# doing-science-to-stuff/ndt

Measured on AMD Instinct MI355X. Metric: Mray/s (primary+shadow+reflect) at 1920x1080, higher is better.
Workload: dtype f64

## Files before the change

### ndt_amd/csrc/ndt_device.hpp

```cpp
#pragma once
#include <hip/hip_runtime.h>
#include <stdint.h>

#define NDT_EPS   (1e-4)
#define NDT_EPS2  ((NDT_EPS) * (NDT_EPS))
#define NDT_INV_EPS2 (1.0 / (NDT_EPS2))
#define NDT_DBL_MAX 1.7976931348623157e308
#define NDT_PI 3.14159265358979323846

#define NDT_DEV __device__ __forceinline__

#define NDT_F_TYPE_MASK   0xff
#define NDT_F_GATE        0x100
#define NDT_F_INF_ENDS    0x200
#define NDT_F_USE_NORMALS 0x400
#define NDT_F_TRANSPARENT 0x800
#define NDT_F_BOX         0x1000
#define NDT_F_FACEBOX     0x2000
#define NDT_F_OBOX        0x4000
#define NDT_F_FACETREE    0x8000
#define NDT_F_FACEGROUPS  0x10000

enum { T_SPHERE = 0, T_HPLANE, T_HDISK, T_CYLINDER, T_HCYLINDER, T_ORTHOTOPE, T_HCUBE, T_HFACET, T_FACET };
enum { NDT_LIGHT_AMBIENT_ = 0, NDT_LIGHT_POINT_ = 1, NDT_LIGHT_DIRECTIONAL_ = 2, NDT_LIGHT_SPOT_ = 3 };
// ... 1116 lines not shown
            } else {
#pragma unroll
                for (int c = 0; c < N; ++c) {
                    w2[c].x = blob[src + 2 * c];
                    w2[c].y = blob[src + 2 * c + 1];
                }
            }
            l_ref[lane] = ref;
            if (has_box) l_ord[lane] = blob[sd.off_oord + id];
            const long long h0 = __double_as_longlong(hdr.x), h1 = __double_as_longlong(hdr.y);
            l_inf[lane] = __longlong_as_double(((h0 >> 32) & 0xffffffffll) | (((h1 & 0xffffll) | ((h1 >> 32) << 16)) << 32));
#pragma unroll
            for (int c = 0; c < N; ++c) *reinterpret_cast<ndt_v2d *>(l_win + lane * 2 * N + 2 * c) = w2[c];
        }
        cls_lds_sync();
        NDT_STAMP(4);
        unsigned long long seen = 0ull;
        if (open && mask.hist_n > 0) {
            for (int k0 = 0; k0 < cnt; k0 += 8) {
                int ids[8];
#pragma unroll
                for (int j = 0; j < 8; ++j) ids[j] = (int)(__double_as_longlong(l_ref[(k0 + j < cnt) ? k0 + j : cnt - 1]) & 0xffffffffll);
                seen |= (unsigned long long)mask.seen_of_8(ids) << k0;
            }
        }
        unsigned long long want = 0ull, any = 0ull;
        if (__ballot(open != 0) != 0ull) {
            unsigned long long todo = (cnt < 64) ? ((1ull << cnt) - 1ull) : ~0ull;
            if (beam) {
                bool keep = true;
                if (lane < cnt && (((int)(__double_as_longlong(l_ref[lane]) >> 32)) & NDT_F_OBOX)) {
                    const unsigned long long ord = (unsigned long long)__double_as_longlong(l_ord[lane]);
                    double t0 = 0.0, t1 = NDT_DBL_MAX;
#pragma unroll
                    for (int k = 0; k < N; ++k) {
                        const int axis = (int)((ord >> (4 * k)) & 15ull);
                        const ndt_v2d box = *reinterpret_cast<const ndt_v2d *>(l_win + lane * 2 * N + 2 * k);
                        const double x0 = l_beam[4 * axis], i0 = l_beam[4 * axis + 1], i1 = l_beam[4 * axis + 2];
                        if (l_beam[4 * axis + 3] != 0.0) {
                            const double a = x0 - box.x, h = box.y;
                            const double p = -h - a, q = h - a;
                            const double c1 = p * i0, c2 = p * i1, c3 = q * i0, c4 = q * i1;
                            const double lo12 = c1 < c2 ? c1 : c2, lo34 = c3 < c4 ? c3 : c4;
                            const double hi12 = c1 < c2 ? c2 : c1, hi34 = c3 < c4 ? c4 : c3;
                            const double lo = lo12 < lo34 ? lo12 : lo34, hi = hi12 > hi34 ? hi12 : hi34;
                            if (lo > t0) t0 = lo;
                            if (hi < t1) t1 = hi;
                        }
                    }
                    keep = t0 <= t1;
                }
                todo &= __ballot(keep);
            }
            while (todo != 0ull) {
                const int k = __ffsll((long long)todo) - 1;
                todo &= todo - 1ull;
                const int flags = __builtin_amdgcn_readfirstlane((int)(__double_as_longlong(l_ref[k]) >> 32));
                bool pass = open != 0;
                if (flags & NDT_F_OBOX) {
                    if (open) pass = item_box_meets<N>(l_win, sd_win, k, box_slot);
                } else if (flags & NDT_F_GATE) {
                    SceneDesc sd_sph = sd;
                    sd_sph.off_bs = k * (2 * N) - k * (N + 2);
                    if (open) pass = bsphere_gate<N>(l_win, sd_sph, k, o, v, min_dist);
                }
                if (pass) want |= 1ull << k;
                if (__ballot(pass && !((seen >> k) & 1ull)) != 0ull) any |= 1ull << k;
            }
            want &= ~seen;
        }
        NDT_STAMP(7);
        int cur = 0;
        auto record_of = [&](int k, int &flags, int &words, int &m, int &at, int &sph) {
            const long long ibits = __double_as_longlong(l_inf[k]);
            const int wm = __builtin_amdgcn_readfirstlane((int)(ibits >> 32));
            at = sd.off_params + __builtin_amdgcn_readfirstlane((int)(ibits & 0xffffffffll));
            words = (wm & 0xffff) + N + 2;
            m = wm >> 16;
            const long long rbits = __double_as_longlong(l_ref[k]);
            flags = __builtin_amdgcn_readfirstlane((int)(rbits >> 32));
            sph = sd.off_bs + __builtin_amdgcn_readfirstlane((int)(rbits & 0xffffffffll)) * (N + 2);
        };
        auto word_of = [&](int j, int words, int at, int sph) {
            return (j < words) ? blob[(j < N + 2) ? sph + j : at + j - (N + 2)] : 0.0;
        };
        auto put = [&](double *buf, int flags, int words, int m, double t0, double t1) {
            if (lane < words) buf[2 + lane] = t0;
            if (lane + 64 < words) buf[2 + 64 + lane] = t1;
            if (lane == 0) {
                buf[0] = __longlong_as_double((long long)(unsigned int)flags);
                buf[1] = __longlong_as_double((long long)m << 32);
            }
        };
        if (any != 0ull) {
            int flags, words, m, at, sph;
            record_of(__ffsll((long long)any) - 1, flags, words, m, at, sph);
            const double t0 = word_of(lane, words, at, sph), t1 = word_of(lane + 64, words, at, sph);
            put(l_par, flags, words, m, t0, t1);
            cls_lds_sync();
        }
        while (any != 0ull) {
            const int k = __ffsll((long long)any) - 1;
            any &= any - 1ull;
            int n_flags = 0, n_words = 0, n_m = 0, n_at = 0, n_sph = 0;
            double t0 = 0.0, t1 = 0.0;
            if (any != 0ull) {
                record_of(__ffsll((long long)any) - 1, n_flags, n_words, n_m, n_at, n_sph);
                t0 = word_of(lane, n_words, n_at, n_sph);
                t1 = word_of(lane + 64, n_words, n_at, n_sph);
            }
            const long long rbits = __double_as_longlong(l_ref[k]);
            const int id = __builtin_amdgcn_readfirstlane((int)(rbits & 0xffffffffll));
            const int flags = __builtin_amdgcn_readfirstlane((int)(rbits >> 32));
            const double *rec = l_par + cur * par_stride;
            bool pass = open != 0 && ((want >> k) & 1ull);
            if ((flags & NDT_F_GATE) && pass) pass = bsphere_gate<N>(rec, sd_par, 0, o, v, min_dist);
            if (pass) {
                double res[N], nrm[N];
                if (isect<N, false>(rec, sd_par, 0, o, v, res, nrm)) {
                    const double dist = v_dist<N>(o, res);
                    if (dist > NDT_EPS && (dist + NDT_EPS < min_dist || min_dist < 0)) {
                        min_dist = dist;
                        best = id;
                    }
                    if (dist_limit == 0.0 || dist < dist_limit) {
                        open = 0;
                        last = id;
                    }
                }
            }
            cur ^= 1;
            if (any != 0ull) put(l_par + cur * par_stride, n_flags, n_words, n_m, t0, t1);
            cls_lds_sync();
            if (__ballot(open != 0) == 0ull) any = 0ull;
        }
        cls_lds_sync();
        NDT_STAMP(2);
        if (open) last = (int)(__double_as_longlong(l_ref[cnt - 1]) & 0xffffffffll);
        cls_lds_sync();
    }
}

#define NDT_KD_STACK 40
#define NDT_STACK_FLAG 0x40000000



struct KdStackLds {
    double *tu;
    int *node;
    int stride;
};

template <int N, int MW, bool LSTACK = false, bool UNI = false>
NDT_DEV void trace_kd(const double *blob, const SceneDesc &sd, VisitMask<MW> &mask, const double (&o)[N],
                      const double (&v)[N], double dist_limit, int &out_obj, int &out_prim
#ifdef NDT_PHASE_TIMING
                      , unsigned long long (&ph)[8], unsigned int (&cnt)[8], unsigned int (&occ)[8]
#endif
                      , KdStackLds ls = KdStackLds{}, ClsLds cl = ClsLds{}, const bool has_ray = true, double *box_slot = nullptr)
{
#ifdef NDT_PHASE_TIMING
    unsigned long long ph_last = __builtin_readcyclecounter();
#endif
#ifdef NDT_T1_KEEP_INV
    constexpr bool KEEP_INV = true;
#else
    constexpr bool KEEP_INV = (MW != 0);
#endif
    auto inv_of = [](double v_i) {
        double r;
        if (v_i < NDT_EPS2 && v_i >= 0.0)
            r = NDT_INV_EPS2;
        else if (v_i > -NDT_EPS2 && v_i <= 0.0)
            r = -NDT_INV_EPS2;
        else
            r = 1.0 / v_i;
        return r;
    };
    double v_inv[N];
    if (KEEP_INV) {
#pragma unroll
        for (int i = 0; i < N; ++i) v_inv[i] = inv_of(v[i]);
    }
    auto inv_at = [&](int dim) {
        if constexpr (KEEP_INV) return v_pick<N>(v_inv, dim);
        else return inv_of(v_pick<N>(v, dim));
    };
    NDT_STAMP(5);

    double t_inf = NDT_DBL_MAX;
    int inf_obj = -1, inf_prim = -1;
    double lt = NDT_DBL_MAX;
    int l_obj = -1, l_prim = -1;

    int st_node[LSTACK ? 1 : NDT_KD_STACK];
    double st_a[LSTACK ? 1 : NDT_KD_STACK], st_tu[LSTACK ? 1 : NDT_KD_STACK];
    int sp = 0;
    int node = 0;
    double ntl = 0, ntu = 0;
    int st = 4;
    bool boxed = false;

    constexpr bool BITS = (MW == 1);
    unsigned long long cand = 0ull;
    int sec = 0, pos = 0, end = 0;
    double min_dist = -1;
    int best_obj = -1, best_prim = -1;
    int sub_i = 0, sub_end = 0, sub_owner = -1, sub_prim = -1;
    long long sub_live = -1;
    double sub_min = -1;

    if (!has_ray) {
        st = 3;
    } else if (sd.n_inf > 0) {
        st = 5;
        if (BITS) {
            cand = sd.inf_bits;
        } else {
            sec = sd.off_inf;
            pos = 0;
            end = sd.n_inf;
        }
    }

    while (true) {
        if (st == 4) {
            double tl = -NDT_DBL_MAX, tu = NDT_DBL_MAX;
            bool box = true;
#pragma unroll
            for (int i = 0; i < N; ++i) {
                if (box) {
                    double v_i = v[i], o_i = o[i];
                    if (!(fabs(v_i) < NDT_EPS2)) {
                        double tl_i = (blob[sd.off_bb + i] - o_i) / v_i;
                        double tu_i = (blob[sd.off_bb + N + i] - o_i) / v_i;
                        if (tl_i > tu_i) {
                            double tmp = tl_i;
                            tl_i = tu_i;
                            tu_i = tmp;
                        }
                        if (tl_i > tl) tl = tl_i;
                        if (tu_i < tu) tu = tu_i;
                        if (tu < -NDT_EPS) box = false;
                    }
                }
            }
            if (box) {
                tl -= NDT_EPS;
                tu += NDT_EPS;
                box = (tu >= -NDT_EPS) && (tl <= tu);
            }
            if (!box || sd.n_kd_nodes <= 0) {
                st = 3;
            } else {
                mask.clear(sd.mask_words);
                if (BITS && sd.gate_bits != 0ull) {
                    unsigned long long todo = sd.gate_bits, dead = 0ull;
                    while (todo != 0ull) {
                        const int id = __ffsll((long long)todo) - 1;
                        todo &= todo - 1ull;
                        const int b = sd.off_bs + id * (N + 2);
                        double c[N], oc[N];
                        blob_vec<N>(blob, b, c);
                        v_sub<N>(o, c, oc);
                        const double oc_len2 = v_dot<N>(oc, oc);
                        const double voc = v_dot<N>(v, oc);
                        const double voc2 = voc * voc;
                        const double desc = voc2 - oc_len2 + blob[b + N + 1];
                        if (desc < 0.0 || (voc > 0.0 && voc2 > desc)) dead |= 1ull << id;
                    }
                    mask.w[0] |= dead;
                }
                node = 0;
                ntl = tl;
                ntu = tu;
                st = 1;
            }
        }
        {
            while (st < 2) {
                NDT_OCC(0);
                if (st == 0) {
                    if (sp == 0) {
                        st = 3;
                    } else {
                        sp -= LSTACK ? ls.stride : 1;
                        double a;
                        if (LSTACK) {
                            const int parent = ls.node[sp];
                            ntu = ls.tu[sp];
                            const ndt_v2d prec = blob_pair(blob, sd.off_kd + 2 * parent);
                            const long long pw0 = __double_as_longlong(prec.x);
                            const int pdim = (int)(pw0 & 0xffffffffll);
                            const double pv_inv = inv_at(pdim);
                            a = (prec.y - v_pick<N>(o, pdim)) * pv_inv;
                            node = (pv_inv < NDT_EPS2) ? parent + 1 : (int)(pw0 >> 32);
                        } else {
                            node = st_node[sp];
                            a = st_a[sp];
                            ntu = st_tu[sp];
                        }
                        ntl = a - NDT_EPS;
                        st = ((lt > a) & !(ntu < 0.0)) ? 1 : 0;
                    }
                } else if (ntu < 0.0) {
                    st = 0;
                }
                if (st == 1) {
                    NDT_COUNT(0);
                    ndt_v2d rec = blob_pair(blob, sd.off_kd + 2 * node);
                    unsigned long long below = ~0ull;
                    if (BITS) {
                        double ns = blob[sd.off_nset + node];
#ifndef NDT_NO_T_HOIST
                        asm volatile("" : "+v"(rec.x), "+v"(rec.y), "+v"(ns));
#endif
                        below = (unsigned long long)__double_as_longlong(ns) & ~mask.w[0];
                    }
                    const long long w0 = __double_as_longlong(rec.x);
                    const int dim = (int)(w0 & 0xffffffffll);
                    if (BITS && below == 0ull) {
                        st = 0;
                    } else if (dim < 0) {
                        if (BITS) {
                            st = 2;
                            cand = below;
                        } else {
                            const long long w1 = __double_as_longlong(rec.y);
                            const int num = (int)(w1 >> 32);
                            st = num > 0 ? 2 : 0;
                            sec = sd.off_leaf;
                            pos = (int)(w1 & 0xffffffffll);
                            end = pos + num;
                        }
                    } else {
                        const double boundary = rec.y;
                        const double v_inv_i = inv_at(dim);
                        const double o_i = v_pick<N>(o, dim);
                        const bool swap = v_inv_i < NDT_EPS2;
                        const int left = node + 1, right = (int)(w0 >> 32);
                        const int near = swap ? right : left, far = swap ? left : right;
                        const double tp = (boundary - o_i) * v_inv_i;
                        const bool alive = lt > ntl;
                        const bool near_only = (ntu < tp - NDT_EPS) & alive;
                        const bool far_only = !near_only & (ntl > tp + NDT_EPS) & alive;
                        const bool both = !near_only & !far_only;
                        if (both & (lt > tp)) {
                            if (LSTACK) { ls.node[sp] = node; ls.tu[sp] = ntu; }
                            else { st_node[sp] = far; st_a[sp] = tp; st_tu[sp] = ntu; }
                            sp += LSTACK ? ls.stride : 1;
                        }
                        const bool go_near = near_only | (both & alive);
                        ntu = (both & alive) ? tp + NDT_EPS : ntu;
                        node = go_near ? near : far;
                        st = (go_near | far_only) ? 1 : 0;
                    }
                }
            }
        }
        NDT_STAMP(0);
        const bool have_list = st == 2 || st == 5, list_is_inf = st == 5;
        if (UNI ? (__ballot(have_list) == 0ull) : !have_list) break;

        min_dist = -1;
        best_obj = -1;
        best_prim = -1;
        bool list_open = have_list;
        bool scanned_together = false;
        if (UNI && MW == 0 && cl.base) {
            const bool elig = have_list && !list_is_inf && mask.hist_n >= 0;
            unsigned long long todo = __ballot(elig);
            const int n_listed = __popcll(__ballot(have_list));
            while (todo != 0ull) {
                const int leader = __ffsll((long long)todo) - 1;
                const int w0 = __builtin_amdgcn_readlane(sec + pos, leader), e0 = __builtin_amdgcn_readlane(sec + end, leader);
                bool mine = elig && sec + pos == w0;
                const unsigned long long group = __ballot(mine);
                todo &= ~group;
                if (__popcll(group) < cl.min_group && !(__popcll(group) == n_listed && n_listed >= 16)) mine = false;
                if (__ballot(mine) == 0ull) continue;
                double md;
                int best, last;
                NDT_STAMP(3);
#ifdef NDT_PHASE_TIMING
                cls_scan<N, MW>(blob, sd, mask, cl.base, mine, o, v, dist_limit, w0, e0, box_slot, boxed, md, best, last, ph, ph_last);
#else
                cls_scan<N, MW>(blob, sd, mask, cl.base, mine, o, v, dist_limit, w0, e0, box_slot, boxed, md, best, last);
#endif
                if (mine) {
                    min_dist = md;
                    best_obj = best;
                    best_prim = best;
                    mask.end_leaf(blob_int(blob, sd.off_kd + 2 * node, 1), last);
                    list_open = false;
                    scanned_together = true;
                }
            }
        }
        int gs = list_open ? 0 : 4;
        while (gs != 4) {
            int prim = -1;
            while (gs < 2) {
                NDT_OCC(1);
                if (gs == 1 && sub_live == 0) {
                    const int oflags = blob_int(blob, sd.off_hdr + 2 * sub_owner, 0);
                    const int first = blob_int(blob, sd.off_hdr + 2 * sub_owner + 1, 0);
                    const bool fresh_hcube = sub_i == first;
                    long long live = -1;
                    int chunk = (sub_i - first) / NDT_HULL_CHUNK;
                    if (oflags & NDT_F_BOX)
                        live = hull_faces<N>(blob, sd.off_params + blob_int(blob, sd.off_hdr + 2 * sub_owner, 1),
                                             (oflags & NDT_F_FACEBOX) != 0, sub_end - first, o, v, chunk, (oflags & NDT_F_FACETREE) != 0,
                                             (oflags & NDT_F_FACEGROUPS) != 0);
                    if (live == 0) {
                        if (fresh_hcube) gs = 0;
                        else sub_i = sub_end;
                        sub_live = -1;
                    } else {
                        const int skip = __ffsll(live) - 1;
                        sub_i = first + ((live == -1) ? 0 : chunk * NDT_HULL_CHUNK) + skip;
                        sub_live = live >> skip;
                    }
                }
                if (gs == 1 && sub_i == sub_end) {
// ... 195 lines not shown
```

### ndt_amd/csrc/ndt_kernels.hip

```cpp
#if NDT_DIMS <= 5 && !defined(NDT_OUTLINE_SMALL)
#define NDT_INLINE_LIBM 1
#endif
#if NDT_DIMS <= 7 && !defined(NDT_OUTLINE_SMALL)
#define NDT_SHADE_INLINE_ISECT 1
#endif
#include "ndt_kernels.hpp"
#include <hip/hip_ext.h>
#include <stdlib.h>
#include <map>
#include <mutex>
#include <tuple>

#ifndef NDT_DIMS
#error "compile with -DNDT_DIMS=<3..10>"
#endif
#define NDT_CAT2(a, b) a##b
#define NDT_CAT(a, b) NDT_CAT2(a, b)

namespace NDT_CAT(ndt_d, NDT_DIMS) {

static constexpr int N = NDT_DIMS;


NDT_DEV int wave_excl_scan(int x, int &total)
// ... 90 lines not shown
        } else if (half_j > 1080 + 45) {
            jp = jp - (1080 + 45);
            eye = 2;
        } else {
            prim_sti<COH>(ws.depth_left + g, 0);
            prim_sti<COH>(ws.hit_obj + g, -1);
            return false;
        }
    }
    const double x = ip / (double)rg.img_w - 0.5;
    const double y = -(jp / y_div - 0.5);
    double pixel[N], temp[N], cam[N];
    blob_vec<N>(blob, sd.off_cam, pos);
    const double focal = blob[sd.off_cam + 4 * N];
    const int ext = sd.off_cam + 4 * N + 8;
    const int cam_type = PLANAR ? 0 : (int)blob[ext];
    if (!PLANAR && cam_type != 0) {
        const double azi = x * blob[ext + 1];
        double view_x, view_y, view_z;
        if (cam_type == 1) {
            const double alt = y * blob[ext + 2];
            view_x = focal * sin(azi) * cos(alt);
            view_y = focal * sin(alt);
            view_z = focal * cos(azi) * cos(alt);
        } else {
            const double y_size = 2.0 * tan(blob[ext + 2] / 2.0) * focal;
            view_x = focal * sin(azi);
            view_y = y * y_size;
            view_z = focal * cos(azi);
        }
        double ax[N];
        v_copy<N>(pixel, pos);
        blob_vec<N>(blob, ext + 3 + 2 * N, ax);
        v_scale<N>(ax, view_x, temp);
        v_add<N>(pixel, temp, pixel);
        blob_vec<N>(blob, ext + 3 + 3 * N, ax);
        v_scale<N>(ax, view_y, temp);
        v_add<N>(pixel, temp, pixel);
        blob_vec<N>(blob, ext + 3 + 4 * N, ax);
        v_scale<N>(ax, view_z, temp);
        v_add<N>(pixel, temp, pixel);
    } else {
        double orig[N], dx[N], dy[N];
        blob_vec<N>(blob, sd.off_cam + N, orig);
        blob_vec<N>(blob, sd.off_cam + 2 * N, dx);
        blob_vec<N>(blob, sd.off_cam + 3 * N, dy);
        v_scale<N>(dx, rg.aspect_w / (double)rg.aspect_h, dx);
        v_copy<N>(pixel, orig);
        v_scale<N>(dx, x, temp);
        v_add<N>(pixel, temp, pixel);
        v_scale<N>(dy, y, temp);
        v_add<N>(pixel, temp, pixel);
        const double screen_dist = v_dist<N>(orig, pos);
        if (screen_dist > NDT_EPS) {
            v_sub<N>(pixel, pos, temp);
            v_scale<N>(temp, focal / screen_dist, temp);
            v_add<N>(pos, temp, pixel);
        }
    }
    v_copy<N>(cam, pos);
    if (eye == 0) blob_vec<N>(blob, ext + 3, cam);
    else if (eye == 2) blob_vec<N>(blob, ext + 3 + N, cam);
    if (!PLANAR && cam_type != 0 && eye != 1) {
        const double azi = x * blob[ext + 1];
        double lx[N], lz[N], bx[N], bz[N], local[N], px[N], pz[N];
        blob_vec<N>(blob, ext + 3 + 2 * N, lx);
        blob_vec<N>(blob, ext + 3 + 4 * N, lz);
        v_proj<N>(lx, lz, temp);
        v_sub<N>(lx, temp, bx);
        v_copy<N>(bz, lz);
        v_unitize<N>(bx);
        v_unitize<N>(bz);
        v_sub<N>(cam, pos, local);
        v_proj<N>(local, bx, px);
        v_proj<N>(local, bz, pz);
        const double vx = v_dot<N>(px, bx), vz = v_dot<N>(pz, bz);
        double rx[N], rz[N];
        v_scale<N>(bx, vx * cos(azi) - vz * sin(azi), rx);
        v_scale<N>(bz, vz * cos(azi) + vx * sin(azi), rz);
        v_sub<N>(cam, px, cam);
        v_sub<N>(cam, pz, cam);
        v_add<N>(cam, rx, cam);
        v_add<N>(cam, rz, cam);
    }
    if (rg.samples && rg.lens) {
        double ax[N];
        blob_vec<N>(blob, ext + 3 + 2 * N, ax);
        v_scale<N>(ax, rg.samples[4 * g + 2], temp);
        v_add<N>(cam, temp, cam);
        blob_vec<N>(blob, ext + 3 + 3 * N, ax);
        v_scale<N>(ax, rg.samples[4 * g + 3], temp);
        v_add<N>(cam, temp, cam);
    }
    v_sub<N>(pixel, cam, look);
    v_unitize<N>(look);
    v_copy<N>(pos, cam);
    {
        const long long at = (g >> 6) * (long long)(N * 64) + (g & 63);
#pragma unroll
        for (int c = 0; c < N; ++c) {
            prim_st<COH>(ws.ray_o + at + c * 64, pos[c]);
            prim_st<COH>(ws.ray_v + at + c * 64, look[c]);
        }
    }
    prim_st<COH>(ws.frac + g, 1.0);
    prim_sti<COH>(ws.depth_left + g, rg.max_depth);
    if (rg.samples && rg.sample_keys) prim_stu<COH>(ws.rng_key + g, rg.sample_keys[g]);
    return true;
}

__global__ void __launch_bounds__(256) k_primary(const double *blob, SceneDesc sd, Workspace ws, RenderGeom rg)
{
    const long long g = (long long)blockIdx.x * blockDim.x + threadIdx.x;
    if (g >= rg.n_primary) return;
    double pos[N], look[N];
    (void)primary_node<false>(blob, sd, ws, rg, g, pos, look);
}



NDT_DEV LevelRange *job_levels_mut(const TraceJob &job) { return const_cast<LevelRange *>(job.levels); }

template <int MW> NDT_DEV void init_visit_mask(VisitMask<MW> &mask, const double *gblob, const SceneDesc &sd, const Workspace &ws)
{
    mask.ext = nullptr;
    mask.ext_stride = 0;
    mask.h0 = mask.h1 = mask.h2 = mask.h3 = 0u;
    mask.hist_n = -1;
    mask.slab_words = sd.mask_words;
    mask.ls.sets = nullptr;
    mask.ls.blob = gblob;
    mask.ls.words = sd.mask_words;
    mask.ls.off_lrange = sd.off_lrange;
    mask.ls.off_leaf = sd.off_leaf;
    mask.ls.cap = sd.hist_cap;
    if (MW == 0) {
        const long long lane_slot = (long long)blockIdx.x * blockDim.x + threadIdx.x;
        mask.ext = ws.mask_slab + lane_slot;
        mask.ext_stride = (int)ws.mask_slab_lanes;
        if (sd.off_lset > 0) mask.ls.sets = reinterpret_cast<const unsigned long long *>(gblob + sd.off_lset);
    }
}

NDT_DEV int seg_light_origin(const double *gblob, const SceneDesc &sd, int s)
{
    unsigned long long rest = ~sd.ambient_bits;
    for (int k = 0; k < s; ++k) rest &= rest - 1ull;
    const int li = __ffsll((long long)rest) - 1;
    const int w = sd.off_lights + li * (6 + 4 * N);
    const int type = blob_int(gblob, w, 0);
    return (type == NDT_LIGHT_POINT_ || type == NDT_LIGHT_SPOT_) ? w + 5 : -1;
}

#ifndef NDT_TICKET_AHEAD
#define NDT_TICKET_AHEAD 256
#endif
template <int MW, bool LDS, bool LSTACK = false, bool PRIM = false>
__global__ void __launch_bounds__(MW == 0 ? NDT_TRACE_T1_MAX_BLOCK : NDT_TRACE_MAX_BLOCK) k_trace(const double *__restrict__ gblob, SceneDesc sd, Workspace ws, TraceJob job)
{
    extern __shared__ __attribute__((aligned(16))) double lds_blob[];
    const double *blob = gblob;
    if (LDS) {
        const int pairs = sd.trace_words >> 1;
        const ndt_v2d *src2 = reinterpret_cast<const ndt_v2d *>(gblob);
        ndt_v2d *dst2 = reinterpret_cast<ndt_v2d *>(lds_blob);
        int i = threadIdx.x;
        for (; i + 3 * (int)blockDim.x < pairs; i += 4 * blockDim.x) {
            const ndt_v2d a = src2[i], b = src2[i + blockDim.x], c = src2[i + 2 * blockDim.x], d = src2[i + 3 * blockDim.x];
            dst2[i] = a; dst2[i + blockDim.x] = b; dst2[i + 2 * blockDim.x] = c; dst2[i + 3 * blockDim.x] = d;
        }
        for (; i < pairs; i += blockDim.x) dst2[i] = src2[i];
        if ((sd.trace_words & 1) && threadIdx.x == 0) lds_blob[sd.trace_words - 1] = gblob[sd.trace_words - 1];
        __syncthreads();
        blob = lds_blob;
    }
    KdStackLds kstack{};
    if (LSTACK) {
        double *base = lds_blob + ((sd.trace_words + 1) & ~1);
        const int depth = sd.kd_depth + 1;
        kstack.stride = blockDim.x;
        kstack.tu = base + threadIdx.x;
        kstack.node = (int *)(base + (size_t)depth * blockDim.x) + threadIdx.x;
    }
    VisitMask<MW> mask;
    init_visit_mask<MW>(mask, gblob, sd, ws);
    ClsLds cls{};
    double *box_slot = nullptr;
    if (MW == 0 && !LDS) {
        const int wave = threadIdx.x >> 6, waves = blockDim.x >> 6;
        const int box_words = sd.off_obox > 0 ? N * 128 : 0;
        if (sd.off_obox > 0) box_slot = lds_blob + (size_t)wave * box_words + 2 * (threadIdx.x & 63);
        if (sd.cls_par_words > 0) {
            cls.base = lds_blob + (size_t)waves * box_words + (size_t)wave * cls_window_words<N>(sd.cls_par_words);
            cls.min_group = sd.cls_min_group;
        }
    }
    const int lane = __lane_id();
    const unsigned int probe_start = job.exit_log ? (unsigned int)wall_clock64() : 0u;
    unsigned int probe_batch = probe_start;
#ifdef NDT_PHASE_TIMING
    unsigned long long ph[8] = { 0, 0, 0, 0, 0, 0, 0, 0 };
    unsigned long long acc[24];
    for (int i = 0; i < 24; ++i) acc[i] = 0ull;
    unsigned long long out_last = __builtin_readcyclecounter();
    unsigned long long batch_mark = 0;
#endif
    const int bs = job.batch;
    const int sh = (bs == 64) ? 6 : (bs == 32) ? 5 : (bs == 16) ? 4 : 3;
    int seg_batches = 0, seg_batches_incl = 0, seg_cnt = 0;
    if (job.n_seg > 0) {
        seg_cnt = (lane < job.n_seg) ? job.seg_count[lane] : 0;
        const int excl = wave_excl_scan((seg_cnt + bs - 1) >> sh, seg_batches);
        seg_batches_incl = excl + ((seg_cnt + bs - 1) >> sh);
    }
    long long dense_count = job.count, dense_begin = job.begin, seg_stride = job.seg_stride;
    if (job.levels) {
        const LevelRange cur = job.levels[job.seg_level];
        seg_stride = cur.seg_stride;
        LevelRange next;
        if (job.publish_level >= 0) {
            next.begin = cur.begin + cur.count;
            next.count = (long long)ws.counters[0] - next.begin;
            next.n_shadow = 0;
            if (next.count < 0 || (ws.counters[2] & 1) != 0) next.count = 0;
            next.seg_stride = (next.count + 63) & ~63LL;
            const bool sh_overflow = (long long)job.n_seg * next.seg_stride > ws.sh_cap;
            if (blockIdx.x == 0 && threadIdx.x < 64) {
                long long emitted = seg_cnt;
                for (int d = 32; d > 0; d >>= 1) emitted += __shfl_xor(emitted, d, 64);
                NDT_SEG_COUNTERS(ws, job.publish_level + 1)[lane] = 0;
                if (lane == 0) {
                    job_levels_mut(job)[job.publish_level].n_shadow = emitted;
                    LevelRange out = next;
                    if (sh_overflow) {
                        atomicOr(&ws.counters[2], 2);
                        const long long need = (long long)job.n_seg * next.seg_stride;
                        ws.counters[3] = need > 0x7fffffffLL ? 0x7fffffff : (int)need;
                        out.count = 0;
                        out.seg_stride = 0;
                    }
                    job_levels_mut(job)[job.publish_level + 1] = out;
                    ws.mail[job.publish_level + 1] = out;
                    __threadfence_system();
                    __hip_atomic_store(&ws.mail_tag[job.publish_level + 1], job.publish_tag, __ATOMIC_RELEASE, __HIP_MEMORY_SCOPE_SYSTEM);
                }
            }
            if (sh_overflow) next.count = 0;
        } else {
            next = job.levels[job.dense_level >= 0 ? job.dense_level : 0];
        }
        if (job.dense_level >= 0) {
            dense_begin = next.begin;
            dense_count = next.count;
        } else {
            dense_count = 0;
        }
    }
    const long long dense_batches = (dense_count + bs - 1) >> sh;
    const long long n_batches = dense_batches + seg_batches;
    const int reserve = ((threadIdx.x >> 6) >= 4) ? job.tail_solo : 0;
    int cur = blockIdx.x % NDT_QUEUE_SHARDS;
    long long last_k = -1;
    bool any_left = true;
    int k_ahead = -1;
    while (true) {
        long long b = -1;
        if (k_ahead >= 0) {
            const int k = __shfl(k_ahead, 0, 64);
            const long long n_here = (n_batches - cur + NDT_QUEUE_SHARDS - 1) / NDT_QUEUE_SHARDS;
            k_ahead = -1;
            if (k < n_here) {
                b = (long long)k * NDT_QUEUE_SHARDS + cur;
                last_k = k;
            }
        }
        while (any_left && b < 0) {
            const long long n_here = (n_batches - cur + NDT_QUEUE_SHARDS - 1) / NDT_QUEUE_SHARDS;
            bool may = true;
            if (reserve > 0 && last_k + 1 + 4 * reserve >= n_here) {
                const int head_cur = __hip_atomic_load(job.queue + cur * NDT_QUEUE_STRIDE, __ATOMIC_RELAXED, __HIP_MEMORY_SCOPE_AGENT);
                may = (long long)head_cur < n_here - reserve;
            }
            if (may) {
                int k = 0;
                if (lane == 0) k = atomicAdd(job.queue + cur * NDT_QUEUE_STRIDE, 1);
                k = __shfl(k, 0, 64);
                if (k < n_here) {
                    b = (long long)k * NDT_QUEUE_SHARDS + cur;
                    last_k = k;
                    break;
                }
            }
            int head = 0x7fffffff;
            if (lane < NDT_QUEUE_SHARDS)
                head = __hip_atomic_load(job.queue + lane * NDT_QUEUE_STRIDE, __ATOMIC_RELAXED, __HIP_MEMORY_SCOPE_AGENT);
            const long long mine = (n_batches - lane + NDT_QUEUE_SHARDS - 1) / NDT_QUEUE_SHARDS - reserve;
            const unsigned long long live = __ballot(lane < NDT_QUEUE_SHARDS && (long long)head < mine);

            if (live == 0ull) {
                any_left = false;
            } else {
                const unsigned long long above = (cur + 1 < 64) ? (live >> (cur + 1)) << (cur + 1) : 0ull;
                cur = __ffsll((long long)(above ? above : live)) - 1;
                last_k = (long long)__shfl(head, cur, 64) - 1;
            }
        }
        if (b < 0) break;
#ifndef NDT_NO_TICKET_AHEAD
        if (MW == 0 && last_k + NDT_TICKET_AHEAD < (n_batches - cur + NDT_QUEUE_SHARDS - 1) / NDT_QUEUE_SHARDS) {
            k_ahead = 0;
            if (lane == 0) k_ahead = atomicAdd(job.queue + cur * NDT_QUEUE_STRIDE, 1);
        }
#endif
        if (job.exit_log) probe_batch = (unsigned int)wall_clock64();
        long long g;
        bool live;
        const bool in_seg = b >= dense_batches;
        int origin_word = -1;
        if (in_seg) {
            const int sb = (int)(b - dense_batches);
            const int s = __popcll(__ballot(lane < job.n_seg && seg_batches_incl <= sb));
            if (MW != 0 && job.seg_light_origins) origin_word = seg_light_origin(gblob, sd, __builtin_amdgcn_readfirstlane(s));
            const int first = (s > 0) ? __shfl(seg_batches_incl, s - 1, 64) : 0;
            const int cnt = __shfl(seg_cnt, s, 64);
            const int idx = (sb - first) * bs + lane;
            live = lane < bs && idx < cnt;
            g = (long long)s * seg_stride + (live ? idx : 0);
        } else {
            const long long r = b * bs + lane;
            live = lane < bs && r < dense_count;
            g = dense_begin + (live ? r : 0);
            if (!PRIM && live && job.dense.valid && job.dense.valid[g] <= 0) live = false;
        }
        double o[N], v[N];
        const bool make = PRIM && !in_seg;
        if (PRIM && make && live) live = primary_node<false, true>(gblob, sd, ws, job.rg, g, o, v);
        if (live || MW == 0) {
        const TracePart &part = in_seg ? job.seg : job.dense;
#ifdef NDT_TRACE_SKIP_KNOB
        if (job.skip_trace == 3) {
            for (int c = 0; c < N; ++c) { o[c] = (double)g; v[c] = 1.0; }
        } else
#endif
        if (live) {
            if (!make) {
                if (origin_word >= 0) blob_vec<N>(gblob, origin_word, o);
                else load_soa<N>(part.o, part.stride, g, o);
                load_soa<N>(part.v, part.stride, g, v);
            }
        } else {
#pragma unroll
            for (int c = 0; c < N; ++c) { o[c] = 0.0; v[c] = 0.0; }
        }
        const double lim = (live && part.lim) ? part.lim[g] : -1.0;
        int obj, prim;
#ifdef NDT_PHASE_TIMING
        unsigned int cnt[8] = { 0, 0, 0, 0, 0, 0, 0, 0 };
        unsigned int occ[8] = { 0, 0, 0, 0, 0, 0, 0, 0 };
        ph[6] += __builtin_readcyclecounter() - out_last;
        batch_mark = wall_clock64();
        if (job.skip_trace) {
            obj = (o[0] + v[0] + lim > 1e300) ? 0 : -1;
            prim = -1;
        } else
        trace_kd<N, MW, LSTACK, MW == 0>(blob, sd, mask, o, v, lim, obj, prim, ph, cnt, occ, kstack, cls, live, box_slot);
        out_last = __builtin_readcyclecounter();
        if (ws.dbg && lane == __ffsll((long long)__ballot(1)) - 1) {
            const unsigned long long now = wall_clock64();
            atomicMax(&ws.dbg[40 + (int)in_seg], now - batch_mark);
            atomicAdd(&ws.dbg[42 + (int)in_seg], now - batch_mark);
            atomicAdd(&ws.dbg[44 + (int)in_seg], 1ull);
        }
        {
            const unsigned long long act = __ballot(1);
            if (lane == __ffsll((long long)act) - 1)
                for (int i = 0; i < 8; ++i) acc[(in_seg ? 16 : 8) + i] += occ[i];
            for (int i = 0; i < 6; ++i) acc[i] += cnt[i];
            acc[6] += 1ull;
            if (ws.dbg) {
                unsigned int nv = cnt[0], ng = cnt[1] + cnt[3], ni = cnt[2] + cnt[4];
                for (int d = 32; d > 0; d >>= 1) {
                    nv = max(nv, (unsigned int)__shfl_xor((int)nv, d, 64));
                    ng = max(ng, (unsigned int)__shfl_xor((int)ng, d, 64));
                    ni = max(ni, (unsigned int)__shfl_xor((int)ni, d, 64));
                }
                if (lane == __ffsll((long long)__ballot(1)) - 1) {
                    atomicMax(&ws.dbg[46], (unsigned long long)nv);
                    atomicMax(&ws.dbg[47], (unsigned long long)ng);
                    atomicMax(&ws.dbg[48], (unsigned long long)ni);
                    atomicMax(&ws.dbg[49], (unsigned long long)occ[0]);
                    atomicMax(&ws.dbg[50], (unsigned long long)occ[2]);
                    atomicMax(&ws.dbg[51], (unsigned long long)occ[4]);
                }
            }
        }
#else
#ifdef NDT_TRACE_SKIP_KNOB
        if (job.skip_trace) {
            obj = (o[0] + v[0] + lim > 1e300) ? 0 : -1;
            prim = -1;
        } else
#endif
        trace_kd<N, MW, LSTACK, MW == 0>(blob, sd, mask, o, v, lim, obj, prim, kstack, cls, live, box_slot);
#endif
#ifdef NDT_TRACE_SKIP_KNOB
        if (job.skip_trace == 2 && obj == -1) live = false;
#endif
        if (live) {
            part.out_obj[g] = obj;
            part.out_prim[g] = prim;
        }
        }
    }
    const unsigned int probe_left = job.exit_log ? (unsigned int)wall_clock64() : 0u;
    if (job.exit_log && lane == 0) {
        const unsigned int w = blockIdx.x * (blockDim.x / 64) + threadIdx.x / 64;
        if (8 * w + 7 < NDT_EXIT_LOG_WORDS) {
            job.exit_log[8 * w] = probe_start;
            job.exit_log[8 * w + 1] = probe_batch;
            job.exit_log[8 * w + 2] = (unsigned int)wall_clock64() | 1u;
            job.exit_log[8 * w + 3] = (__builtin_amdgcn_s_getreg((31 << 11) | 4) & 0xffffffu) | ((blockDim.x / 64) << 24);
            job.exit_log[8 * w + 4] = probe_left | 1u;
        }
    }
#ifdef NDT_PHASE_TIMING
    ph[6] += __builtin_readcyclecounter() - out_last;
    if (ws.dbg) {
        for (int i = 0; i < 24; ++i) {
            unsigned long long x = acc[i];
            for (int d = 32; d > 0; d >>= 1) x += __shfl_xor(x, d, 64);
            if (lane == 0 && x) atomicAdd(&ws.dbg[8 + i], x);
        }
        if (lane == 0) {
            for (int i = 0; i < 4; ++i) atomicAdd(&ws.dbg[i], ph[i]);
            atomicAdd(&ws.dbg[7], ph[7]);
            atomicAdd(&ws.dbg[32], ph[4]);
            atomicAdd(&ws.dbg[4], 1ull);
            atomicAdd(&ws.dbg[5], ph[5]);
            atomicAdd(&ws.dbg[6], ph[6]);
        }
    }
#endif
}

#if defined(NDT_PHASE_TIMING) || defined(NDT_TRACE_SKIP_KNOB)
static int env_int(const char *name, int def)
{
    const char *e = getenv(name);
    return (e && *e) ? atoi(e) : def;
}
#else
static constexpr int env_int(const char *, int def) { return def; }
#endif

template <typename K> static int resident_blocks(K kernel, int block, size_t lds)
{
    static std::mutex mu;
    static std::map<std::tuple<int, const void *, int, size_t>, int> known;
    int dev = 0;
    (void)hipGetDevice(&dev);
    const auto key = std::make_tuple(dev, reinterpret_cast<const void *>(kernel), block, lds);
    std::lock_guard<std::mutex> lock(mu);
    auto it = known.find(key);
    if (it != known.end()) return it->second;
    int per_cu = 0;
    if (hipOccupancyMaxActiveBlocksPerMultiprocessor(&per_cu, kernel, block, lds) != hipSuccess || per_cu < 1) per_cu = 1;
    int cus = 256, v = 0;
    if (hipDeviceGetAttribute(&v, hipDeviceAttributeMultiprocessorCount, dev) == hipSuccess && v > 0) cus = v;
    known[key] = per_cu * cus;
    return per_cu * cus;
}

#define NDT_LAUNCH_TRACE(kernel, grid, block, lds)                                                             \
    do {                                                                                                       \
        if (ev_start)                                                                                          \
            hipExtLaunchKernelGGL((kernel), dim3((unsigned)(grid)), dim3(block), (std::uint32_t)(lds), s, ev_start, ev_stop, 0u, blob, sd, ws, job); \
        else                                                                                                   \
            hipLaunchKernelGGL((kernel), dim3((unsigned)(grid)), dim3(block), lds, s, blob, sd, ws, job);      \
    } while (0)
typedef void (*TraceKernel)(const double *, SceneDesc, Workspace, TraceJob);
static void launch_trace(hipStream_t s, const double *blob, SceneDesc sd, Workspace ws, TraceJob job, int tier,
                         int mask_words, hipEvent_t ev_start, hipEvent_t ev_stop)
{
    if (job.count <= 0 && job.n_seg <= 0) {
        if (ev_start) {
            (void)hipEventRecord(ev_start, s);
            (void)hipEventRecord(ev_stop, s);
        }
        return;
    }
    static const int block = env_int("NDT_TRACE_BLOCK", NDT_TRACE_BLOCK);
    static const int force_batch = env_int("NDT_TRACE_BATCH", 0);
    job.batch = 64;
    job.skip_trace = env_int("NDT_TRACE_SKIP", 0);
    {
        static const int tail_solo = env_int("NDT_TRACE_TAIL_SOLO", 16);
        job.tail_solo = tail_solo > 0 ? tail_solo : 0;
    }
    if (force_batch == 64 || force_batch == 32 || force_batch == 16 || force_batch == 8) job.batch = force_batch;
    const long long upper = job.count + (job.n_seg > 0 ? job.seg_stride * job.n_seg : 0);
    long long blocks = (upper + job.batch * (block / 64) - 1) / (job.batch * (block / 64));
    if (tier == 0) {
        static const int extra_lds = env_int("NDT_TRACE_EXTRA_LDS", 0);
        const size_t lds = (size_t)sd.trace_words * sizeof(double) + (size_t)extra_lds;
        static const int lstack_full = env_int("NDT_TRACE_LSTACK", NDT_TRACE_MAX_BLOCK);
        static const int small_launch = env_int("NDT_TRACE_SMALL", 4096);
        int lstack_block = lstack_full;
        if (lstack_full >= 256 && upper / job.batch < small_launch) lstack_block = 256;
        const size_t lds_stack = ((size_t)((sd.trace_words + 1) & ~1) * 8) + (size_t)lstack_block * (sd.kd_depth + 1) * 12;
        const bool prim = job.make_primaries != 0;
        if (lstack_block >= 64 && mask_words <= 1 && lds_stack <= 160 * 1024) {
            const TraceKernel kern = prim ? k_trace<1, true, true, true> : k_trace<1, true, true>;
            const int res = resident_blocks(kern, lstack_block, lds_stack);
            long long nb = (upper + job.batch * (lstack_block / 64) - 1) / (job.batch * (lstack_block / 64));
            if (nb > res) nb = res;
            NDT_LAUNCH_TRACE(kern, nb, lstack_block, lds_stack);
        } else if (lstack_block >= 64 && mask_words > 1 && lds_stack <= 160 * 1024) {
            const TraceKernel kern = prim ? k_trace<NDT_MASK_REG_WORDS, true, true, true> : k_trace<NDT_MASK_REG_WORDS, true, true>;
            const int res = resident_blocks(kern, lstack_block, lds_stack);
            long long nb = (upper + job.batch * (lstack_block / 64) - 1) / (job.batch * (lstack_block / 64));
            if (nb > res) nb = res;
            NDT_LAUNCH_TRACE(kern, nb, lstack_block, lds_stack);
        } else if (mask_words <= 1) {
            const TraceKernel kern = prim ? k_trace<1, true, false, true> : k_trace<1, true>;
            const int res = resident_blocks(kern, block, lds);
            if (blocks > res) blocks = res;
            NDT_LAUNCH_TRACE(kern, blocks, block, lds);
        } else {
            const TraceKernel kern = prim ? k_trace<NDT_MASK_REG_WORDS, true, false, true> : k_trace<NDT_MASK_REG_WORDS, true>;
            const int res = resident_blocks(kern, block, lds);
            if (blocks > res) blocks = res;
            NDT_LAUNCH_TRACE(kern, blocks, block, lds);
        }
    } else {
        const TraceKernel kern_t1 = job.make_primaries ? k_trace<0, false, false, true> : k_trace<0, false>;
        const size_t lds = (size_t)(block / 64) * ((sd.off_obox > 0 ? N * 128 : 0) + (sd.cls_par_words > 0 ? cls_window_words<N>(sd.cls_par_words) : 0)) * sizeof(double);
        const int res = resident_blocks(kern_t1, block, lds);
        if (blocks > res) blocks = res;
        const long long max_blocks = ws.mask_slab_lanes / block;
        if (blocks > max_blocks) blocks = max_blocks;
        NDT_LAUNCH_TRACE(kern_t1, blocks, block, lds);
    }
}

#ifndef NDT_SHADE_WAVES
#define NDT_SHADE_WAVES 2
#endif

struct VecPair {
    double a[N], b[N];
};
#if NDT_DIMS >= 6 && !defined(NDT_STREAM_INLINE_ISECT)
#define NDT_HAVE_ISECT_CALL 1
__device__ __attribute__((noinline)) VecPair isect_full_call(const double *blob, const SceneDesc *sd, int prim, VecPair ray)
{
    VecPair out;
#pragma unroll
    for (int c = 0; c < N; ++c) { out.a[c] = 0.0; out.b[c] = 0.0; }
    isect<N, true>(blob, *sd, prim, ray.a, ray.b, out.a, out.b);
    return out;
}
NDT_DEV void isect_full_outlined(const double *blob, const SceneDesc *sd, int prim, const double (&o)[N], const double (&v)[N],
                                 double (&hit)[N], double (&nrm)[N])
{
    VecPair ray;
#pragma unroll
    for (int c = 0; c < N; ++c) { ray.a[c] = o[c]; ray.b[c] = v[c]; }
    const VecPair out = isect_full_call(blob, sd, prim, ray);
#pragma unroll
    for (int c = 0; c < N; ++c) { hit[c] = out.a[c]; nrm[c] = out.b[c]; }
}
#endif
NDT_DEV void isect_full(const double *blob, const SceneDesc *sd, int prim, const double (&o)[N], const double (&v)[N], double (&hit)[N],
                        double (&nrm)[N])
{
#if defined(NDT_SHADE_INLINE_ISECT) || !defined(NDT_HAVE_ISECT_CALL)
    isect<N, true>(blob, *sd, prim, o, v, hit, nrm);
#else
    isect_full_outlined(blob, sd, prim, o, v, hit, nrm);
#endif
}
NDT_DEV void isect_full_stream(const double *blob, const SceneDesc *sd, int prim, const double (&o)[N], const double (&v)[N],
                               double (&hit)[N], double (&nrm)[N])
{
#ifdef NDT_HAVE_ISECT_CALL
    isect_full_outlined(blob, sd, prim, o, v, hit, nrm);
#else
    isect<N, true>(blob, *sd, prim, o, v, hit, nrm);
#endif
}



#ifdef NDT_PHASE_TIMING
#define NDT_SEC_BEGIN() unsigned long long sec_t[8] = { 0, 0, 0, 0, 0, 0, 0, 0 }; unsigned long long sec_last = wall_clock64(); const unsigned long long sec_first = sec_last
#define NDT_SEC(k) do { const unsigned long long now_ = wall_clock64(); sec_t[k] += now_ - sec_last; sec_last = now_; } while (0)
// ... 649 lines not shown
```

Baseline: 4441.

## Reload trace kernargs on demand, hoist segment light origins, and defer inverse-direction compute

Adds per-instantiation knobs for the trace kernel. It can re-read job and workspace fields directly from the kernarg segment where they are used, rather than keeping them live in SGPRs across the loop. It can compute each lane's segment light origin once per wave and fetch it with readlane instead of recomputing it per batch. It can also defer the inverse ray direction computation into the kd traversal reset, hidden behind an asm barrier. The goal is lower register pressure and less repeated scalar work in the hot loop, at the cost of extra scalar loads and more template complexity.

```diff
diff --git a/ndt_amd/csrc/ndt_device.hpp b/ndt_amd/csrc/ndt_device.hpp
--- a/ndt_amd/csrc/ndt_device.hpp
+++ b/ndt_amd/csrc/ndt_device.hpp
@@ -1292,7 +1292,7 @@
     int stride;
 };
 
-template <int N, int MW, bool LSTACK = false, bool UNI = false>
+template <int N, int MW, bool LSTACK = false, bool UNI = false, bool LAZY_INV = false>
 NDT_DEV void trace_kd(const double *blob, const SceneDesc &sd, VisitMask<MW> &mask, const double (&o)[N],
                       const double (&v)[N], double dist_limit, int &out_obj, int &out_prim
 #ifdef NDT_PHASE_TIMING
@@ -1319,7 +1319,7 @@
         return r;
     };
     double v_inv[N];
-    if (KEEP_INV) {
+    if (KEEP_INV && !LAZY_INV) {
 #pragma unroll
         for (int i = 0; i < N; ++i) v_inv[i] = inv_of(v[i]);
     }
@@ -1411,6 +1411,14 @@
                         if (desc < 0.0 || (voc > 0.0 && voc2 > desc)) dead |= 1ull << id;
                     }
                     mask.w[0] |= dead;
+                }
+                if (KEEP_INV && LAZY_INV) {
+#pragma unroll
+                    for (int i = 0; i < N; ++i) {
+                        double v_i = v[i];
+                        asm volatile("" : "+v"(v_i));
+                        v_inv[i] = inv_of(v_i);
+                    }
                 }
                 node = 0;
                 ntl = tl;
diff --git a/ndt_amd/csrc/ndt_kernels.hip b/ndt_amd/csrc/ndt_kernels.hip
--- a/ndt_amd/csrc/ndt_kernels.hip
+++ b/ndt_amd/csrc/ndt_kernels.hip
@@ -266,12 +266,82 @@
     return (type == NDT_LIGHT_POINT_ || type == NDT_LIGHT_SPOT_) ? w + 5 : -1;
 }
 
+typedef __attribute__((address_space(4))) const char *KernargBytes;
+struct TraceKernargs {
+    const double *gblob;
+    SceneDesc sd;
+    Workspace ws;
+    TraceJob job;
+};
+constexpr size_t KARG_TRACE_WS = offsetof(TraceKernargs, ws);
+constexpr size_t KARG_TRACE_JOB = offsetof(TraceKernargs, job);
+#ifdef NDT_HEAD_STEPS
+constexpr int trace_head_steps(int, int mw, bool, bool) { return mw != 0 ? (NDT_HEAD_STEPS) : 0; }
+#else
+constexpr int trace_head_steps(int n, int mw, bool lstack, bool prim)
+{
+    if (mw == 0) return 0;
+    if (prim) return 7;
+    if (n == 4 && mw == 4 && lstack) return 5;
+    if (n == 4 && mw == 1 && !lstack) return 0;
+    if (n == 5 && lstack) return 5;
+    if (n == 6 && mw == 1 && !lstack) return 0;
+    if (n == 8 && mw == 1 && !lstack) return 1;
+    if (n == 10 && !lstack) return 5;
+    if (n == 11 && !(mw == 1 && lstack)) return 0;
+    return 7;
+}
+#endif
+NDT_DEV KernargBytes karg_here()
+{
+    KernargBytes p = (KernargBytes)__builtin_amdgcn_kernarg_segment_ptr();
+    asm volatile("" : "+s"(p));
+    return p;
+}
+template <typename T> NDT_DEV T karg_get(KernargBytes p)
+{
+    static_assert(sizeof(T) % 4 == 0 && std::is_trivially_copyable<T>::value, "words");
+    union { T v; unsigned int w[sizeof(T) / 4]; } u;
+#pragma unroll
+    for (size_t i = 0; i < sizeof(T) / 4; ++i) u.w[i] = reinterpret_cast<__attribute__((address_space(4))) const unsigned int *>(p)[i];
+    return u.v;
+}
+#define NDT_KARG_PTR(obj, base, member) \
+    (obj).member = *reinterpret_cast<__attribute__((address_space(4))) decltype((obj).member) const *>((base) + offsetof(decltype(obj), member))
+NDT_DEV TracePart karg_trace_part(bool in_seg)
+{
+    const int at = in_seg ? (int)offsetof(TraceJob, seg) : (int)offsetof(TraceJob, dense);
+    const KernargBytes kp = karg_here() + KARG_TRACE_JOB + __builtin_amdgcn_readfirstlane(at);
+    TracePart p = karg_get<TracePart>(kp);
+    NDT_KARG_PTR(p, kp, o); NDT_KARG_PTR(p, kp, v); NDT_KARG_PTR(p, kp, lim); NDT_KARG_PTR(p, kp, valid);
+    NDT_KARG_PTR(p, kp, out_obj); NDT_KARG_PTR(p, kp, out_prim);
+    return p;
+}
+NDT_DEV Workspace karg_trace_workspace(KernargBytes ka)
+{
+    const KernargBytes kp = ka + KARG_TRACE_WS;
+    Workspace w = karg_get<Workspace>(kp);
+    NDT_KARG_PTR(w, kp, ray_o); NDT_KARG_PTR(w, kp, ray_v); NDT_KARG_PTR(w, kp, frac); NDT_KARG_PTR(w, kp, depth_left);
+    NDT_KARG_PTR(w, kp, hit_obj); NDT_KARG_PTR(w, kp, child_refl); NDT_KARG_PTR(w, kp, child_refr); NDT_KARG_PTR(w, kp, sh_mask);
+    NDT_KARG_PTR(w, kp, count); NDT_KARG_PTR(w, kp, rng_key);
+    return w;
+}
+NDT_DEV RenderGeom karg_trace_geom(KernargBytes ka)
+{
+    const KernargBytes kp = ka + KARG_TRACE_JOB + offsetof(TraceJob, rg);
+    RenderGeom rg = karg_get<RenderGeom>(kp);
+    NDT_KARG_PTR(rg, kp, samples); NDT_KARG_PTR(rg, kp, sample_keys);
+    return rg;
+}
+
 #ifndef NDT_TICKET_AHEAD
 #define NDT_TICKET_AHEAD 256
 #endif
 template <int MW, bool LDS, bool LSTACK = false, bool PRIM = false>
 __global__ void __launch_bounds__(MW == 0 ? NDT_TRACE_T1_MAX_BLOCK : NDT_TRACE_MAX_BLOCK) k_trace(const double *__restrict__ gblob, SceneDesc sd, Workspace ws, TraceJob job)
 {
+    constexpr int STEPS = trace_head_steps(N, MW, LSTACK, PRIM);
+    constexpr bool KARG = (STEPS & 1) != 0, SEG_ONCE = (STEPS & 2) != 0, LAZY = (STEPS & 4) != 0;
     extern __shared__ __attribute__((aligned(16))) double lds_blob[];
     const double *blob = gblob;
     if (LDS) {
@@ -322,10 +392,12 @@
     const int bs = job.batch;
     const int sh = (bs == 64) ? 6 : (bs == 32) ? 5 : (bs == 16) ? 4 : 3;
     int seg_batches = 0, seg_batches_incl = 0, seg_cnt = 0;
+    int seg_origin = -1;
     if (job.n_seg > 0) {
         seg_cnt = (lane < job.n_seg) ? job.seg_count[lane] : 0;
         const int excl = wave_excl_scan((seg_cnt + bs - 1) >> sh, seg_batches);
         seg_batches_incl = excl + ((seg_cnt + bs - 1) >> sh);
+        if (SEG_ONCE && job.seg_light_origins && seg_cnt > 0) seg_origin = seg_light_origin(gblob, sd, lane);
     }
     long long dense_count = job.count, dense_begin = job.begin, seg_stride = job.seg_stride;
     if (job.levels) {
@@ -434,7 +506,8 @@
         if (in_seg) {
             const int sb = (int)(b - dense_batches);
             const int s = __popcll(__ballot(lane < job.n_seg && seg_batches_incl <= sb));
-            if (MW != 0 && job.seg_light_origins) origin_word = seg_light_origin(gblob, sd, __builtin_amdgcn_readfirstlane(s));
+            if (SEG_ONCE) origin_word = __builtin_amdgcn_readlane(seg_origin, __builtin_amdgcn_readfirstlane(s));
+            else if (MW != 0 && job.seg_light_origins) origin_word = seg_light_origin(gblob, sd, __builtin_amdgcn_readfirstlane(s));
             const int first = (s > 0) ? __shfl(seg_batches_incl, s - 1, 64) : 0;
             const int cnt = __shfl(seg_cnt, s, 64);
             const int idx = (sb - first) * bs + lane;
@@ -444,13 +517,28 @@
             const long long r = b * bs + lane;
             live = lane < bs && r < dense_count;
             g = dense_begin + (live ? r : 0);
-            if (!PRIM && live && job.dense.valid && job.dense.valid[g] <= 0) live = false;
+            if constexpr (KARG) {
+                if (!PRIM && live) {
+                    const int *valid = karg_trace_part(false).valid;
+                    if (valid && valid[g] <= 0) live = false;
+                }
+            } else {
+                if (!PRIM && live && job.dense.valid && job.dense.valid[g] <= 0) live = false;
+            }
         }
         double o[N], v[N];
         const bool make = PRIM && !in_seg;
-        if (PRIM && make && live) live = primary_node<false, true>(gblob, sd, ws, job.rg, g, o, v);
+        if (PRIM && make && live) {
+            if (KARG) {
+                const KernargBytes ka = karg_here();
+                live = primary_node<false, true>(gblob, sd, karg_trace_workspace(ka), karg_trace_geom(ka), g, o, v);
+            } else {
+                live = primary_node<false, true>(gblob, sd, ws, job.rg, g, o, v);
+            }
+        }
         if (live || MW == 0) {
-        const TracePart &part = in_seg ? job.seg : job.dense;
+        const TracePart part_here = KARG ? karg_trace_part(in_seg) : TracePart{};
+        const TracePart &part = KARG ? part_here : in_seg ? job.seg : job.dense;
 #ifdef NDT_TRACE_SKIP_KNOB
         if (job.skip_trace == 3) {
             for (int c = 0; c < N; ++c) { o[c] = (double)g; v[c] = 1.0; }
@@ -477,7 +565,7 @@
             obj = (o[0] + v[0] + lim > 1e300) ? 0 : -1;
             prim = -1;
         } else
-        trace_kd<N, MW, LSTACK, MW == 0>(blob, sd, mask, o, v, lim, obj, prim, ph, cnt, occ, kstack, cls, live, box_slot);
+        trace_kd<N, MW, LSTACK, MW == 0, LAZY>(blob, sd, mask, o, v, lim, obj, prim, ph, cnt, occ, kstack, cls, live, box_slot);
         out_last = __builtin_readcyclecounter();
         if (ws.dbg && lane == __ffsll((long long)__ballot(1)) - 1) {
             const unsigned long long now = wall_clock64();
@@ -515,14 +603,16 @@
             prim = -1;
         } else
 #endif
-        trace_kd<N, MW, LSTACK, MW == 0>(blob, sd, mask, o, v, lim, obj, prim, kstack, cls, live, box_slot);
+        trace_kd<N, MW, LSTACK, MW == 0, LAZY>(blob, sd, mask, o, v, lim, obj, prim, kstack, cls, live, box_slot);
 #endif
 #ifdef NDT_TRACE_SKIP_KNOB
         if (job.skip_trace == 2 && obj == -1) live = false;
 #endif
         if (live) {
-            part.out_obj[g] = obj;
-            part.out_prim[g] = prim;
+            const TracePart out_here = KARG ? karg_trace_part(in_seg) : TracePart{};
+            const TracePart &out = KARG ? out_here : part;
+            out.out_obj[g] = obj;
+            out.out_prim[g] = prim;
         }
         }
     }
@@ -556,6 +646,9 @@
     }
 #endif
 }
+
+static_assert(std::is_same<decltype(&k_trace<1, true, true, false>), void (*)(const double *, SceneDesc, Workspace, TraceJob)>::value,
+              "k_trace's parameters changed: change TraceKernargs with them");
 
 #if defined(NDT_PHASE_TIMING) || defined(NDT_TRACE_SKIP_KNOB)
 static int env_int(const char *name, int def)
```

Result: faster. 4513, median of 6 (+1.6%).
